# Accustomer/CUDA-AKAZE

Hardware: AMD Instinct MI355X
Metric: pairs_per_sec_detect_describe_match_1080p (higher is better)
Workload: dtype f32; 1 GPU; configs[1]: 1920x1080 grayscale pairs, 4 octaves x 4 sublevels, PM_G2, MLDB-486, max_pts 10000, float path; detect+describe both images + match, D2H included; pairs_per_launch_sequence=256, distinct_pairs_per_gpu=16, float_sequences_enqueued=77, octave_streams=one stream per context, step_pipeline=2, rank0_gpu_numa_node=1

## Files before the change

cuda-akaze_amd/akaze_hip/__init__.py:

```python
import ctypes as C
import os

import numpy as np

try:
    import torch as _torch
except ImportError:
    _torch = None

_HERE = os.path.dirname(os.path.abspath(__file__))
LIB_PATH = os.environ.get("HAK_LIB") or os.path.join(os.path.dirname(_HERE), "libhipakaze.so")

FLEN = 61
MAX_DIST = 96
PM_G1, PM_G2, WEICKERT, CHARBONNIER = 0, 1, 2, 3

POINT_DTYPE = np.dtype([
    ("x", "<f4"), ("y", "<f4"), ("octave", "<i4"), ("response", "<f4"), ("size", "<f4"), ("angle", "<f4"),
    ("features", "u1", (FLEN,)), ("_pad", "u1", (3,)),
    ("match", "<i4"), ("distance", "<i4"), ("match_x", "<f4"), ("match_y", "<f4"),
])
assert POINT_DTYPE.itemsize == 104
MATCH_PAIR_DTYPE = np.dtype([("query", "<i4"), ("train", "<i4"), ("distance", "<i4"), ("second", "<i4"),
                             ("x1", "<f4"), ("y1", "<f4"), ("x2", "<f4"), ("y2", "<f4")])
# ... 99 lines not shown
    "hak_memcpy_h2d": (C.c_int, [_vp, _vp, C.c_long]),
    "hak_fed_tau": (C.c_int, [C.c_float, C.c_int, C.c_float, C.c_int, _fp, C.c_int]),
    "hak_gauss_taps": (None, [C.c_float, C.c_int, _fp]),
    "hak_compare_indices": (None, [_ip, _ip]),
    "hak_describe_plan_query": (C.c_int, [C.c_int, C.POINTER(C.c_uint), C.POINTER(C.c_uint)]),
    "hak_query_schedule": (C.c_int, [_vp, _ip, _ip, _fp, _fp]),
    "hak_query_geometry": (C.c_int, [_vp, _ip]),
    "hak_query_traffic": (C.c_int, [_vp, C.c_int, C.POINTER(hak_traffic)]),
    "hak_prof_enable": (C.c_int, [_vp, C.c_int]),
    "hak_prof_read": (C.c_int, [_vp, C.c_int, C.POINTER(C.c_double), _ip]),
    "hak_prof_reset": (C.c_int, [_vp]),
}
TEST_SYMBOLS = {
    "hak_debug_plane": (C.c_int, [_vp, C.c_int, C.c_int, C.c_int, C.c_int, _vp]),
    "hak_debug_kcontrast": (C.c_int, [_vp, C.c_int, _fp]),
    "hak_op_lowpass": (C.c_int, [_vp, _vp, C.c_int, C.c_int, C.c_int, C.c_float, C.c_int]),
    "hak_op_down_smooth": (C.c_int, [_vp, _vp, _vp, C.c_int, C.c_int, C.c_int, C.c_int, C.c_int, C.c_int]),
    "hak_op_kcontrast": (C.c_int, [_vp, C.c_int, C.c_int, C.c_int, C.c_float, _fp, _fp, _ip]),
    "hak_op_flow": (C.c_int, [_vp, _vp, C.c_int, C.c_int, C.c_int, C.c_int, C.c_float]),
    "hak_op_nld_steps": (C.c_int, [_vp, _vp, _vp, _vp, C.c_int, C.c_int, C.c_int, _fp, C.c_int]),
    "hak_op_nld_steps_batch": (C.c_int, [_vp, _vp, _vp, _vp, C.c_long, C.c_int, C.c_int, C.c_int, C.c_int, _fp, C.c_int]),
    "hak_op_fed_cycle": (C.c_int, [_vp, C.c_int, C.c_int, C.c_int, C.c_int, _vp, _vp, _vp, _vp, C.c_long, C.c_int, C.c_int, C.c_int, C.c_int,
                                   _fp, _fp, C.c_int]),
    "hak_op_rcp_check": (C.c_int, [C.c_uint, C.c_uint, C.POINTER(C.c_ulonglong)]),
    "hak_op_smooth_flow": (C.c_int, [_vp, _vp, _vp, C.c_int, C.c_int, C.c_int, C.c_int, C.c_float]),
    "hak_op_hessian": (C.c_int, [_vp, _vp, _vp, _vp, C.c_int, C.c_int, C.c_int, C.c_int]),
    "hak_op_fast_conv_u8": (C.c_int, [_vp, C.c_int, _vp, C.c_int, C.c_int, C.c_int, C.c_float, C.c_int]),
    "hak_op_fast_lowpass": (C.c_int, [_vp, _vp, C.c_int, C.c_int, C.c_int, C.c_float, C.c_int]),
    "hak_op_fast_base": (C.c_int, [_vp, C.c_int, _vp, C.c_int, C.c_int, C.c_int, C.c_float, C.c_int, C.c_float, _ip, _ip, _ip, _ip]),
    "hak_op_fast_down_smooth": (C.c_int, [_vp, _vp, _vp, C.c_int, C.c_int, C.c_int, C.c_int, C.c_int, C.c_int]),
    "hak_op_fast_kcontrast": (C.c_int, [_vp, C.c_int, C.c_int, C.c_int, C.c_float, _ip, _ip, _ip]),
    "hak_op_fast_flow": (C.c_int, [_vp, _vp, C.c_int, C.c_int, C.c_int, C.c_int, C.c_int]),
    "hak_op_fast_smooth_flow": (C.c_int, [_vp, _vp, _vp, C.c_int, C.c_int, C.c_int, C.c_int, C.c_int]),
    "hak_op_fast_nld_steps": (C.c_int, [_vp, _vp, _vp, _vp, C.c_int, C.c_int, C.c_int, _fp, C.c_int]),
    "hak_op_fast_nld_steps_batch": (C.c_int, [_vp, _vp, _vp, _vp, C.c_long, C.c_int, C.c_int, C.c_int, C.c_int, _fp, C.c_int]),
    "hak_op_fast_fed_cycle": (C.c_int, [_vp, C.c_int, C.c_int, C.c_int, C.c_int, _vp, _vp, _vp, _vp, C.c_long, C.c_int, C.c_int, C.c_int,
                                        C.c_int, _ip, _fp, C.c_int]),
    "hak_op_fast_level_tile": (C.c_int, [_vp, C.c_int, C.c_int, C.c_int, C.c_int, _vp, _vp, _vp, C.c_long, C.c_int, C.c_int, C.c_int,
                                         C.c_int, C.c_int, _ip, _fp, C.c_int, _ip]),
    "hak_op_fast_hessian": (C.c_int, [_vp, _vp, _vp, _vp, C.c_int, C.c_int, C.c_int, C.c_int, _ip]),
    "hak_op_hessian_batch": (C.c_int, [_vp, _vp, _vp, _vp, C.c_int, C.c_int, C.c_int, C.c_int, C.c_int, _ip]),
    "hak_op_fast_hessian_batch": (C.c_int, [_vp, _vp, _vp, _vp, C.c_int, C.c_int, C.c_int, C.c_int, C.c_int, _ip]),
    "hak_debug_set_plane": (C.c_int, [_vp, C.c_int, C.c_int, C.c_int, C.c_int, _vp]),
    "hak_op_tail_begin": (C.c_int, [_vp]),
    "hak_op_tail_level": (C.c_int, [_vp, C.c_int, C.c_int, _vp]),
    "hak_op_tail_det_level": (C.c_int, [_vp, C.c_int, C.c_int, _vp]),
# ... 24 lines not shown


class _Libs:

    def __init__(self):
        self.product = C.CDLL(LIB_PATH, mode=C.RTLD_GLOBAL)
        self.test = None
        for name, (res, args) in SYMBOLS.items():
            try:
                f = getattr(self.product, name)
            except AttributeError:
                if os.environ.get("HAK_LIB"):
                    continue
                raise
            f.restype, f.argtypes = res, args
            setattr(self, name, f)

    def load_test(self):
        if self.test is None:
            if not os.path.exists(TEST_LIB_PATH):
                raise ImportError(f"{TEST_LIB_PATH} is missing: build it with `make -C cuda-akaze_amd/csrc`")
            self.test = C.CDLL(TEST_LIB_PATH)
            for name, (res, args) in TEST_SYMBOLS.items():
                f = getattr(self.test, name)
                f.restype, f.argtypes = res, args
                setattr(self, name, f)
        return self.test

    def __getattr__(self, name):
        if name in TEST_SYMBOLS:
            self.load_test()
            return self.__dict__[name]
        raise AttributeError(name)


lib = _Libs()


def check(status):
    if status != 0:
        raise HakError(lib.hak_last_error().decode() or f"libhipakaze status {status}")


def iAlignUp(a, b):
    return a - a % b + b if a % b else a


# ... 484 lines not shown
```

cuda-akaze_amd/csrc/hak_internal.h:

```cpp
#pragma once
#include <cstdlib>
#include <hip/hip_runtime.h>
#include <stdint.h>
#include "../../include/hipakaze.h"
#include "hak_knobs.h"

#define HAK_NBINS 300
#define HAK_WAVE 64

struct HakOct {
    int w, h, p;
    long plane;
};

struct HakLayout {
    int noct, ms;
    HakOct oct[HAK_MAX_OCTAVES];
    long lvl_off[HAK_MAX_OCTAVES];
    long smooth_off[HAK_MAX_OCTAVES], flow_off[HAK_MAX_OCTAVES], tmp_off[HAK_MAX_OCTAVES];
    long arena;

    __host__ __device__ long lt(int o, int s) const { return lvl_off[o] + (long)s * oct[o].plane; }
    __host__ __device__ long dxy(int o, int s) const { return lvl_off[o] + (long)(ms + 2 * s) * oct[o].plane; }
};
// ... 342 lines not shown
                          bool* hess_done = nullptr, float fixed_ikc = 0.f);
int hak_launch_level_tile(hipStream_t st, const int* src, HakOct so, bool head, int* smooth, int* dst, int* tmp, long stride,
                          HakOct dd, int nimg, const int* taps, int diffusivity, const float* tau, int n,
                          const HakImgState* state, int octave, int* dxy = nullptr, int step = 0, const HakBatch* b = nullptr,
                          const HakLayout* L = nullptr, const HakTables* htab = nullptr, int sub = 0, int idthreshold = 0, bool* hess_done = nullptr);
int hak_launch_rcp_check(unsigned lo, unsigned hi, unsigned long long* d_bad);
static inline bool hak_fed_sf_covers(const HakKnobs& kn, int diffusivity, const HakOct& dd, int nimg, const HakOct* so = nullptr)
{
    if (!hak_stream_pays(kn.fuse_sf, dd.w, dd.h, nimg) || diffusivity != HAK_PM_G2 || (dd.w & 3) != 0 || dd.w < 16 || dd.h < 8) return false;
    return !so || (kn.fuse_head && !(so->w & 1) && !(so->h & 1));
}
bool hak_launch_fed_sf_head(hipStream_t st, const float* src, HakOct so, float* smooth, float* flow, float* dst, long stride,
                            HakOct dd, int nimg, const float* taps, int diffusivity, const float* tau, int ns,
                            const HakImgState* state, int octave, bool write_g);
bool hak_launch_fed_sf_head(hipStream_t st, const int* src, HakOct so, int* smooth, int* flow, int* dst, long stride,
                            HakOct dd, int nimg, const int* taps, int diffusivity, const float* tau, int ns,
                            const HakImgState* state, int octave, bool write_g);
bool hak_launch_fed_sf(hipStream_t st, const float* src, float* smooth, float* flow, float* dst, long stride,
                       int w, int h, int p, int nimg, const float* taps, int diffusivity, const float* tau, int ns,
                       const HakImgState* state, int octave, bool write_g, bool store_smooth = true, float fixed_ikc = 0.f);
bool hak_launch_fed_sf(hipStream_t st, const int* src, int* smooth, int* flow, int* dst, long stride,
                       int w, int h, int p, int nimg, const int* taps, int diffusivity, const float* tau, int ns,
                       const HakImgState* state, int octave, bool write_g);
int hak_fed_groups(int n, int max_fuse, int w, bool wide_only);
bool hak_fed_wide_only(int octave, int w);
int hak_fed_group_size(int n, int G, int g);
void hak_launch_fed_group(hipStream_t st, const float* src, const float* flow, float* dst, long stride,
                          int w, int h, int p, int nimg, const float* tau, int ns);
void hak_launch_fed_group(hipStream_t st, const int* src, const int* flow, int* dst, long stride,
                          int w, int h, int p, int nimg, const float* tau, int ns);
void hak_launch_derivate(hipStream_t st, const float* src, float* dxy, long stride, int w, int h, int p, int nimg, int step);
void hak_launch_derivate(hipStream_t st, const int* src, int* dxy, long stride, int w, int h, int p, int nimg, int step);
void hak_launch_hessian(hipStream_t st, const float* dxy, float* det, long stride, int w, int h, int p, int nimg, int step);
void hak_launch_hessian(hipStream_t st, const int* dxy, int* det, long stride, int w, int h, int p, int nimg, int step);
void hak_deriv_factors(float* fac1, float* fac2);
template <typename V> static inline void hak_deriv_factors_as(V& f1, V& f2)
{
    float a, b;
    hak_deriv_factors(&a, &b);
    f1 = hak_fac_as(a, V());
    f2 = hak_fac_as(b, V());
}
void hak_launch_deinterleave(hipStream_t st, const float* ab, float* a, float* b, int w, int h, int p);

void hak_launch_ingest_u8(hipStream_t st, const unsigned char* src, long src_stride, int sp, float* dst, long dst_stride,
                          int dp, int w, int h, int nimg);
// ... 214 lines not shown
```

cuda-akaze_amd/csrc/hak_knobs.h:

```cpp
#pragma once
#include "../../include/hipakaze.h"

#define HAK_FED_MAX_FUSE 8

struct HakKnobs {
    int hess_stream = 1;
    int base_stream = 1;
    int base_hist = 0;
    int hess_cbuf = 256;
    int desc_order = 4;
    int desc_plan = 1;
    int desc_sort = 1;
    int hess_lp = 0;
    int level_tile = 1;
    int level_hess = 1;
    int level_min_steps = 8;
    int level_min_blocks = 96;
    int fuse_sf = 1;
    int fuse_head = 1;
    int max_fuse = 8;
    int hist_min_blocks = 256;
    int hist_rpb_max = 8;
    int hess_side = 0;
    int spine_max_px = 0;
    int side_streams = HAK_MAX_OCTAVES;
    int graph_pads = 1;
    int tail_fork = 1;
    int graph = 1;
    int serial = 0;
    int null_order = 1;
    int timing = 0;
    int prof_fence = 0;
    int stream_min_waves = 2048;
    int download_blocks = 128;
};
HakKnobs hak_knobs_from_env();
const HakKnobs& hak_process_knobs();

struct HakMatchKnobs {
    int valu = 0;
    int qt = 1;
    int slices = 0;
};
// ... 2 lines not shown
```

cuda-akaze_amd/csrc/hak_knobs.hip:

```cpp
#include "hak_knobs.h"
#include <climits>
#include <cstdlib>

static int env_int(const char* name, int dflt, int lo = INT_MIN, int hi = INT_MAX)
{
    const char* e = getenv(name);
    if (!e) return dflt;
    const long v = strtol(e, nullptr, 10);
    return v < lo ? lo : (v > hi ? hi : (int)v);
}

HakKnobs hak_knobs_from_env()
{
    static const struct { const char* name; int HakKnobs::*field; int lo, hi; } rows[] = {
        {"HAK_HESS_STREAM", &HakKnobs::hess_stream, INT_MIN, INT_MAX},
        {"HAK_BASE_STREAM", &HakKnobs::base_stream, INT_MIN, INT_MAX},
        {"HAK_BASE_HIST", &HakKnobs::base_hist, INT_MIN, INT_MAX},
        {"HAK_HESS_CBUF", &HakKnobs::hess_cbuf, 1, 256},
        {"HAK_DESC_ORDER", &HakKnobs::desc_order, 0, 255},
        {"HAK_DESC_PLAN", &HakKnobs::desc_plan, INT_MIN, INT_MAX},
        {"HAK_DESC_SORT", &HakKnobs::desc_sort, INT_MIN, INT_MAX},
        {"HAK_HESS_LP", &HakKnobs::hess_lp, INT_MIN, INT_MAX},
        {"HAK_LEVEL_TILE", &HakKnobs::level_tile, INT_MIN, INT_MAX},
        {"HAK_LEVEL_HESS", &HakKnobs::level_hess, INT_MIN, INT_MAX},
        {"HAK_LEVEL_MIN_STEPS", &HakKnobs::level_min_steps, INT_MIN, INT_MAX},
        {"HAK_LEVEL_MIN_BLOCKS", &HakKnobs::level_min_blocks, 1, INT_MAX},
        {"HAK_FUSE_SF", &HakKnobs::fuse_sf, INT_MIN, INT_MAX},
        {"HAK_FUSE_HEAD", &HakKnobs::fuse_head, INT_MIN, INT_MAX},
        {"HAK_FED_MAX_FUSE", &HakKnobs::max_fuse, 1, HAK_FED_MAX_FUSE},
        {"HAK_HIST_MIN_BLOCKS", &HakKnobs::hist_min_blocks, 1, INT_MAX},
        {"HAK_HIST_RPB_MAX", &HakKnobs::hist_rpb_max, 1, INT_MAX},
        {"HAK_HESS_SIDE", &HakKnobs::hess_side, INT_MIN, INT_MAX},
        {"HAK_SPINE_MAX_PX", &HakKnobs::spine_max_px, INT_MIN, INT_MAX},
        {"HAK_SIDE_STREAMS", &HakKnobs::side_streams, 1, INT_MAX},
        {"HAK_GRAPH_PADS", &HakKnobs::graph_pads, INT_MIN, INT_MAX},
        {"HAK_TAIL_FORK", &HakKnobs::tail_fork, INT_MIN, INT_MAX},
        {"HAK_GRAPH", &HakKnobs::graph, INT_MIN, INT_MAX},
        {"HAK_SERIAL", &HakKnobs::serial, INT_MIN, INT_MAX},
        {"HAK_NULL_ORDER", &HakKnobs::null_order, INT_MIN, INT_MAX},
        {"HAK_TIMING", &HakKnobs::timing, INT_MIN, INT_MAX},
        {"HAK_PROF_FENCE", &HakKnobs::prof_fence, INT_MIN, INT_MAX},
        {"HAK_STREAM_MIN_WAVES", &HakKnobs::stream_min_waves, 1, INT_MAX},
        {"HAK_DOWNLOAD_BLOCKS", &HakKnobs::download_blocks, 1, INT_MAX},
    };
    HakKnobs k;
    for (const auto& r : rows) k.*r.field = env_int(r.name, k.*r.field, r.lo, r.hi);
    return k;
}

const HakKnobs& hak_process_knobs()
{
    static const HakKnobs k = hak_knobs_from_env();
// ... 12 lines not shown
```

cuda-akaze_amd/csrc/hak_sequence.hip:

```cpp
#include "hak_internal.h"
#include <cstdio>
#include <cstring>
#include <string>
#include <type_traits>

#include "hak_ctx.h"

static thread_local const char* g_launch_err = nullptr;
void hak_note_launch_error(const char* msg) { if (!g_launch_err) g_launch_err = msg; }

void order_after_null_stream(hak_ctx* c, hipStream_t st)
{
    if (!c || !c->null_order || !c->ev_null || st == nullptr) return;
    const hipError_t q = hipStreamQuery(nullptr);
    if (q == hipSuccess) return;
    (void)hipGetLastError();
    if (hipEventRecord(c->ev_null, nullptr) != hipSuccess || hipStreamWaitEvent(st, c->ev_null, 0) != hipSuccess) (void)hipGetLastError();
}

void maps_guard_begin(hak_ctx* c)
{
    if (c->maps_dirty) {
        const size_t h = c->L.oct[0].h, words = (c->L.oct[0].w + 63) / 64, B = c->cfg.batch;
        (void)hipMemsetAsync(c->maps, 0, sizeof(unsigned long long) * (size_t)c->L.oct[0].plane * B, c->stream);
// ... 71 lines not shown
        const auto* img = static_cast<const std::conditional_t<is_fast<V>, unsigned char, float>*>(a.images);
        const V* taps_base = taps_of<V>(c->taps_base, c->itaps_base);
        const bool based = hak_launch_base_level(st, img, a.image_stride, a.pitch, Lt, tmp, S, oc.w, oc.h, oc.p, nimg, taps1, taps_base, c->base_R,
                                                 c->state, cfg.per, L.noct, kn);
        if constexpr (is_fast<V>) {
            if (!based) {
                hak_launch_lowpass(st, img, a.image_stride, a.pitch, smooth, S, oc.w, oc.h, oc.p, nimg, taps1, 2);
                hak_launch_contrast(st, smooth, S, oc.w, oc.h, oc.p, nimg, c->state, cfg.per, L.noct);
                hak_launch_lowpass(st, img, a.image_stride, a.pitch, Lt, S, oc.w, oc.h, oc.p, nimg, taps_base, c->base_R);
            }
        } else (void)based;
        return;
    }
    const int n = lp.nsteps;
    if (level_tile_pays(c, oc, nimg) && (is_fast<V> || s == 0 || n >= kn.level_min_steps || kn.level_tile == 2)) {
        ProfScope ps(pc, HAK_PROF_FED, st);
        const int nl = hak_launch_level_tile(st, s == 0 ? A + L.lt(o - 1, 0) : A + L.lt(o, s - 1), s == 0 ? L.oct[o - 1] : oc, s == 0, smooth, Lt, tmp, S,
                                             oc, nimg, taps1, cfg.diffusivity, lp.tau.data(), n, c->state, o,
                                             kn.level_hess ? A + L.dxy(o, s) : nullptr, lp.sigma_size, &a.b, &L, &c->htab, s, dthreshold_of<V>(c),
                                             &a.hess_fused[o * HAK_MAX_SCALES + s]);
        count_fed(nl, (s == 0 ? 1.0 * L.oct[o - 1].w * L.oct[o - 1].h : 4.0 * oc.w * oc.h) + 8.0 * oc.w * oc.h + (nl - 1) * 12.0 * oc.w * oc.h);
        return;
    }
    const int G = hak_fed_groups(n, is_fast<V> && kn.max_fuse > 4 ? 4 : kn.max_fuse, oc.w, hak_fed_wide_only(o, oc.w));
    const int ns0 = hak_fed_group_size(n, G, 0);
    V* dst0 = (G % 2 == 1) ? Lt : tmp;
    const V* fsrc;
    bool fused_first = false;
    if (s == 0) {
        if (hak_fed_sf_covers(kn, cfg.diffusivity, oc, nimg, &L.oct[o - 1])) {
            ProfScope ps(pc, HAK_PROF_FED, st);
            fused_first = hak_launch_fed_sf_head(st, A + L.lt(o - 1, 0), L.oct[o - 1], smooth, flow, dst0, S, oc, nimg, taps1, cfg.diffusivity,
                                                 lp.tau.data(), ns0, c->state, o, G > 1);
            if (fused_first) count_fed(1, 2.0 * L.oct[o - 1].w * L.oct[o - 1].h + (G > 1 ? 12.0 : 8.0) * oc.w * oc.h);
        }
        V* first = (G % 2 == 0) ? Lt : tmp;
        if (!fused_first) {
            { ProfScope ps(pc, HAK_PROF_DOWN, st);
              hak_launch_down_smooth(st, A + L.lt(o - 1, 0), first, smooth, S, L.oct[o - 1], oc, nimg, taps1); }
            ProfScope ps(pc, HAK_PROF_FLOW, st);
            hak_launch_flow(st, smooth, flow, S, oc.w, oc.h, oc.p, nimg, cfg.diffusivity, c->state, o);
        }
        fsrc = first;
    } else {
        fsrc = A + L.lt(o, s - 1);
        if (hak_fed_sf_covers(kn, cfg.diffusivity, oc, nimg)) {
// ... 253 lines not shown
```

cuda-akaze_amd/csrc/hak_test_api.hip:

```cpp
#include "hak_ctx.h"
#include "../../include/hipakaze_test.h"
#include <cmath>
#include <cstdio>
#include <cstring>
#include <type_traits>

extern "C" int hak_debug_plane(hak_ctx* c, int img, int kind, int o, int s, float* h_dst)
{
    if (!c || img < 0 || img >= c->cfg.batch || o < 0 || o >= c->L.noct || s < 0 || s >= c->L.ms) return fail("bad plane");
    const HakLayout& L = c->L;
    const HakOct oc = L.oct[o];
    HIP_TRY(hipStreamSynchronize(c->stream));
    const float* arena = c->arena + (long)img * L.arena;
    if (kind == HAK_PLANE_LT) {
        HIP_TRY(hipMemcpy2D(h_dst, sizeof(float) * oc.w, arena + L.lt(o, s), sizeof(float) * oc.p, sizeof(float) * oc.w, oc.h, hipMemcpyDeviceToHost));
        return 0;
    }
    float* tmp = nullptr;
    HIP_TRY(hipMalloc((void**)&tmp, sizeof(float) * 2 * (size_t)oc.plane));
    int rc = 0;
    const float* src = tmp;
    if (kind == HAK_PLANE_DET) {
        const int step = c->plan[(size_t)o * L.ms + s].sigma_size;
        if (c->last_fast) hak_launch_hessian(nullptr, reinterpret_cast<const int*>(arena + L.dxy(o, s)), reinterpret_cast<int*>(tmp), 0, oc.w, oc.h, oc.p, 1, step);
// ... 221 lines not shown
    if (nsteps < 1 || nimg < 1 || !kcontrast) return fail("nsteps < 1, nimg < 1 or no contrast factors");
    if (p % 4 || stride % 4 || (op_fast<V> && head && sp % 4)) return fail("pitch and stride must be multiples of 4");
    HakImgState* state = nullptr;
    if (op_state<V>(&state, kcontrast, nimg)) return 1;
    V taps[8];
    op_taps<V>(1.f, 2, taps);
    const int G = hak_fed_groups(nsteps, op_max_fuse<V>(), w, false);
    const int ns0 = hak_fed_group_size(nsteps, G, 0);
    V* dst0 = (G % 2 == 1) ? dst : tmp;
    int rc = 0;
    const bool ok = head ? hak_launch_fed_sf_head(nullptr, src, HakOct{sw, sh, sp, (long)sh * sp}, smooth, flow, dst0, stride,
                                                  HakOct{w, h, p, (long)h * p}, nimg, taps, HAK_PM_G2, tau, ns0, state, 0, G > 1)
                         : hak_launch_fed_sf(nullptr, src, smooth, flow, dst0, stride, w, h, p, nimg, taps, HAK_PM_G2, tau, ns0, state, 0, G > 1);
    if (!ok) rc = fail(std::string(who) + ": k_fed_sf does not cover this case");
    else op_fed_groups<V>(dst0, flow, dst, tmp, stride, w, h, p, nimg, tau, nsteps, G, 1, ns0);
    const hipError_t e = hipDeviceSynchronize();
    if (e != hipSuccess && !rc) rc = fail(std::string(who) + ": " + (op_fast<V> ? hipGetErrorString(e) : "kernel"));
    (void)hipFree(state);
    return rc;
}
extern "C" int hak_op_fed_cycle(const float* src, int head, int sw, int sh, int sp, float* smooth, float* flow, float* dst, float* tmp,
                                long stride, int w, int h, int p, int nimg, const float* kcontrast, const float* tau, int nsteps)
{ return fed_cycle_t("hak_op_fed_cycle", src, head, sw, sh, sp, smooth, flow, dst, tmp, stride, w, h, p, nimg, kcontrast, tau, nsteps); }
extern "C" int hak_op_fast_fed_cycle(const int* src, int head, int sw, int sh, int sp, int* smooth, int* flow, int* dst, int* tmp,
                                     long stride, int w, int h, int p, int nimg, const int* kcontrast, const float* tau, int nsteps)
{ return fed_cycle_t("hak_op_fast_fed_cycle", src, head, sw, sh, sp, smooth, flow, dst, tmp, stride, w, h, p, nimg, kcontrast, tau, nsteps); }

extern "C" int hak_op_fast_base(const unsigned char* img, int sp, int* lt, int w, int h, int p, float var_base, int radius, float per,
                                int* kc, int* hmax, int* hist, int* route)
{
    if (radius < 1 || radius > 5) return fail("radius must be 1..5");
    if (p % 4) return fail("pitch must be a multiple of 4");
    int taps1[8], tapsb[8];
    op_taps<int>(1.f, 2, taps1);
    op_taps<int>(var_base, radius, tapsb);
    const HakKnobs kn = hak_knobs_from_env();
    const size_t plane = (size_t)h * p;
    int* buf = nullptr;
    HIP_TRY(hipMalloc((void**)&buf, sizeof(int) * 3 * plane));
    HakImgState* st = nullptr;
    if (hipMalloc((void**)&st, sizeof(HakImgState)) != hipSuccess) { (void)hipFree(buf); return fail("state alloc"); }
    (void)hipMemset(st, 0, sizeof(HakImgState));
    hak_launch_reset_state(nullptr, st, 1);
    int *Lt = buf, *grad = buf + plane, *smooth = buf + 2 * plane;
    const bool based = hak_launch_base_level(nullptr, img, 0, sp, Lt, grad, 0, w, h, p, 1, taps1, tapsb, radius, st, per, 1, kn);
    if (!based) {
// ... 393 lines not shown
```

cuda-akaze_amd/csrc/kernels_fedsf.hip:

```cpp
#include "fed_common.h"

#ifndef HAK_FS_PD
#define HAK_FS_PD 3
#endif
#ifndef HAK_FS_PD_MAXNS
#define HAK_FS_PD_MAXNS 4
#endif

namespace {

template <typename V, int NS>
struct FsState {
    static constexpr int W = fed_lane_px(NS);
    using Px = FedPx<V, W>;
    static constexpr int GS = fed_gsum_slots(NS);
    static constexpr int UF = fed_unroll(NS);
    static constexpr int PD = NS <= HAK_FS_PD_MAXNS ? HAK_FS_PD : 3;
    Px Lr[6];
    Px Rp[6];
    Px Sm[3];
    V SmL[3], SmR[3];
    Px Lw[NS][2];
    Px Qw[NS][2];
    GHrow<V, W> GH[GS];
    Px GV[GS];
    Px gprev;
    Px Lq[PD];
};

template <bool DEC, typename V, int W>
__device__ __forceinline__ FedPx<V, W> fs_fetch(const V* __restrict__ L, const int row, const int lp, const int xl, const int sh)
{
    if constexpr (!DEC) return px_load<V, W>(L + (long)row * lp + xl);
    else {
        const V* r = L + (long)min(2 * row, sh - 1) * lp + min(2 * xl, lp - 2 * W);
        FedPx<V, W> o;
#pragma unroll
        for (int i = 0; i < W / 2; i++) {
            const FedPx<V, 4> a = px_load<V, 4>(r + 4 * i);
            o.e[2 * i] = a.e[0];
            o.e[2 * i + 1] = a.e[2];
        }
        return o;
    }
}

struct FsOut { __amdgpu_buffer_rsrc_t r; unsigned smo, go; };

template <typename V, int NS, int U, bool YEDGE, bool XE, bool WRITE_G, bool DEC, bool WRITE_SM>
__device__ __forceinline__ void fs_iter(FsState<V, NS>& S, const int t, const V* __restrict__ L, V* __restrict__ D, const int p,
                                        const int xl, const int x0, const int w, const int h, const int ybeg, const int yend,
                                        const bool owns, const FedFacs<V, NS>& fac, const SfTaps<V> kk, const float ikc,
                                        const int lp, const int sh, const FsOut& O)
{
    constexpr int W = FsState<V, NS>::W, GS = FsState<V, NS>::GS, PD = FsState<V, NS>::PD;
    using Px = FedPx<V, W>;
    const bool le = x0 == 0, re = x0 + W - 1 == w - 1;
    {
        const Px Lc = S.Lq[pmod(U, PD)];
        S.Lr[pmod(U, 6)] = Lc;
        S.Lq[pmod(U, PD)] = fs_fetch<DEC, V, W>(L, min(t + PD, h - 1), lp, xl, sh);
    }
    {
        const Px c = S.Lr[pmod(U, 6)];
        V a[W + 4];
        a[0] = wave_shr1(c.e[W - 2]); a[1] = wave_shr1(c.e[W - 1]);
#pragma unroll
        for (int j = 0; j < W; j++) a[2 + j] = c.e[j];
        a[W + 2] = wave_shl1(c.e[0]); a[W + 3] = wave_shl1(c.e[1]);
        if (XE) {
            a[1] = le ? a[3] : a[1];
            a[0] = le ? a[4] : a[0];
            if constexpr (!DEC) {
                a[W + 2] = re ? a[W] : a[W + 2];
                a[W + 3] = re ? a[W - 1] : a[W + 3];
            } else {
                a[W + 2] = re ? a[W + 1] : a[W + 2];
                a[W + 3] = re ? a[W] : a[W + 3];
            }
        }
        Px rp;
#pragma unroll
        for (int j = 0; j < W; j++) rp.e[j] = hak_conv5(a[j + 2], a[j + 1], a[j + 3], a[j], a[j + 4], kk);
        S.Rp[pmod(U, 6)] = rp;
        if (YEDGE) {
            S.Rp[pmod(U - 2, 6)] = px_sel(t == 1, rp, S.Rp[pmod(U - 2, 6)]);
            S.Rp[pmod(U - 4, 6)] = px_sel(t == 2, rp, S.Rp[pmod(U - 4, 6)]);
            if constexpr (!DEC) {
                S.Rp[pmod(U, 6)] = px_sel(t == h, S.Rp[pmod(U - 2, 6)], S.Rp[pmod(U, 6)]);
                S.Rp[pmod(U, 6)] = px_sel(t == h + 1, S.Rp[pmod(U - 4, 6)], S.Rp[pmod(U, 6)]);
            } else {
                S.Rp[pmod(U, 6)] = px_sel(t == h, S.Rp[pmod(U - 1, 6)], S.Rp[pmod(U, 6)]);
                S.Rp[pmod(U, 6)] = px_sel(t == h + 1, S.Rp[pmod(U - 3, 6)], S.Rp[pmod(U, 6)]);
            }
        }
    }
    {
        const int a = t - 2;
        const Px c = S.Rp[pmod(U - 2, 6)], u1 = S.Rp[pmod(U - 3, 6)], d1 = S.Rp[pmod(U - 1, 6)];
        const Px u2 = S.Rp[pmod(U - 4, 6)], d2 = S.Rp[pmod(U, 6)];
        Px sm;
#pragma unroll
        for (int j = 0; j < W; j++) sm.e[j] = hak_conv5(c.e[j], u1.e[j], d1.e[j], u2.e[j], d2.e[j], kk);
        if constexpr (WRITE_SM)
            px_buf_store_nt(O.r, O.smo + (a >= ybeg && a < yend ? (unsigned)(a * p) * (unsigned)sizeof(V) : HAK_BUF_OOB), sm);
        V sl = wave_shr1(sm.e[W - 1]), sr = wave_shl1(sm.e[0]);
        if (XE) {
            sl = le ? sm.e[1] : sl;
            sr = re ? sm.e[W - 2] : sr;
        }
        S.Sm[pmod(U, 3)] = sm; S.SmL[pmod(U, 3)] = sl; S.SmR[pmod(U, 3)] = sr;
        if (YEDGE && a == 1) { S.Sm[pmod(U - 2, 3)] = sm; S.SmL[pmod(U - 2, 3)] = sl; S.SmR[pmod(U - 2, 3)] = sr; }
        if (YEDGE && a == h) {
            S.Sm[pmod(U, 3)] = S.Sm[pmod(U - 2, 3)]; S.SmL[pmod(U, 3)] = S.SmL[pmod(U - 2, 3)]; S.SmR[pmod(U, 3)] = S.SmR[pmod(U - 2, 3)];
        }
    }
    const int tf = t - 3;
    {
        V su[W + 2], sc[W + 2], sd[W + 2];
        su[0] = S.SmL[pmod(U - 2, 3)]; su[W + 1] = S.SmR[pmod(U - 2, 3)];
        sc[0] = S.SmL[pmod(U - 1, 3)]; sc[W + 1] = S.SmR[pmod(U - 1, 3)];
        sd[0] = S.SmL[pmod(U, 3)]; sd[W + 1] = S.SmR[pmod(U, 3)];
#pragma unroll
        for (int j = 0; j < W; j++) {
            su[j + 1] = S.Sm[pmod(U - 2, 3)].e[j];
            sc[j + 1] = S.Sm[pmod(U - 1, 3)].e[j];
            sd[j + 1] = S.Sm[pmod(U, 3)].e[j];
        }
        float den[W];
        bool fast = true;
#pragma unroll
        for (int j = 0; j < W; j++) {
            V dx, dy;
            hak_scharr(su[j], su[j + 1], su[j + 2], sc[j], sc[j + 2], sd[j], sd[j + 1], sd[j + 2], dx, dy);
            den[j] = 1.f + hak_dif2(dx, dy, ikc);
            fast = fast && den[j] < 0x1p64f;
        }
        Px g;
        if (__ballot(!fast) == 0ull) {
#pragma unroll
            for (int j = 0; j < W; j++) g.e[j] = hak_g_as<V>(hak_rcp_newton(den[j]));
        } else {
#pragma unroll
            for (int j = 0; j < W; j++) g.e[j] = hak_g_as<V>(1.f / den[j]);
        }
        if (WRITE_G) px_buf_store_nt(O.r, O.go + (tf >= ybeg && tf < yend ? (unsigned)(tf * p) * (unsigned)sizeof(V) : HAK_BUF_OOB), g);
        S.GH[pmod(U, GS)] = fed_gh(g);
        S.GV[pmod(U - 1, GS)] = px_add(S.gprev, g);
        S.gprev = g;
    }
#pragma unroll
    for (int k = 1; k <= NS; k++) {
        const int rho = tf - k;
        const Px Lc = k == 1 ? S.Lr[pmod(U - 3 - 1, 6)] : S.Lw[k - 1][pmod(U - k, 2)];
        const Px Ls = k == 1 ? S.Lr[pmod(U - 3, 6)] : S.Lw[k - 1][pmod(U - k + 1, 2)];
        Px Qn = fed_q(S.GV[pmod(U - k, GS)], Ls, Lc);
        Px Qp = S.Qw[k - 1][pmod(U - k - 1, 2)];
        if (YEDGE) {
            Qp = px_sel(rho == 0, px_neg(Qn), Qp);
            Qn = px_sel(rho == h - 1, px_neg(Qp), Qn);
        }
        S.Qw[k - 1][pmod(U - k, 2)] = Qn;
        const Px out = fed_row<XE>(Lc, S.GH[pmod(U - k, GS)], Qn, Qp, x0, w, fac.f[k - 1]);
        if (k < NS) {
            S.Lw[k < NS ? k : 0][pmod(U - k, 2)] = out;
        } else if (rho >= ybeg && rho < yend && owns) {
            px_store_nt(D + (long)rho * p + x0, out);
        }
// ... 143 lines not shown
    return true;
}

__global__ __launch_bounds__(256) void k_rcp_check(unsigned lo, unsigned hi, unsigned long long* bad)
{
    unsigned long long n = 0;
    for (unsigned long long b = lo + blockIdx.x * (unsigned long long)blockDim.x + threadIdx.x; b < hi;
         b += (unsigned long long)gridDim.x * blockDim.x) {
        const float d = __uint_as_float((unsigned)b);
        n += __float_as_uint(hak_rcp_newton(d)) != __float_as_uint(1.0f / d);
    }
    if (n) atomicAdd(bad, n);
}

template <typename V>
bool launch_fed_sf_head_t(hipStream_t st, const V* src, HakOct so, V* smooth, V* flow, V* dst, long stride, HakOct dd, int nimg,
                          const V* taps, int diffusivity, const float* tau, int ns, const HakImgState* state, int octave, bool write_g)
{
    if ((so.w & 1) || (so.h & 1) || so.p < 2 * 8 || dd.w != so.w / 2 || dd.h != so.h / 2) return false;
    return launch_fs_any<V>(st, src, smooth, flow, dst, stride, dd.w, dd.h, dd.p, nimg, SfTaps<V>{taps[0], taps[1], taps[2]},
                            diffusivity, tau, ns, state, octave, 0.f, write_g, so.p, so.h);
}

}

int hak_launch_rcp_check(unsigned lo, unsigned hi, unsigned long long* d_bad)
{
    k_rcp_check<<<4096, 256>>>(lo, hi, d_bad);
    return hipGetLastError() == hipSuccess ? 0 : 1;
}

bool hak_launch_fed_sf(hipStream_t st, const float* src, float* smooth, float* flow, float* dst, long stride,
                       int w, int h, int p, int nimg, const float* taps, int diffusivity, const float* tau, int ns,
                       const HakImgState* state, int octave, bool write_g, bool store_smooth, float fixed_ikc)
{ return launch_fs_any<float>(st, src, store_smooth ? smooth : nullptr, flow, dst, stride, w, h, p, nimg, SfTaps<float>{taps[0], taps[1], taps[2]},
                                diffusivity, tau, ns, state, octave, fixed_ikc, write_g); }
bool hak_launch_fed_sf(hipStream_t st, const int* src, int* smooth, int* flow, int* dst, long stride,
                       int w, int h, int p, int nimg, const int* taps, int diffusivity, const float* tau, int ns,
                       const HakImgState* state, int octave, bool write_g)
{ return launch_fs_any<int>(st, src, smooth, flow, dst, stride, w, h, p, nimg, SfTaps<int>{taps[0], taps[1], taps[2]},
                              diffusivity, tau, ns, state, octave, 0.f, write_g); }

bool hak_launch_fed_sf_head(hipStream_t st, const float* src, HakOct so, float* smooth, float* flow, float* dst, long stride,
                            HakOct dd, int nimg, const float* taps, int diffusivity, const float* tau, int ns,
                            const HakImgState* state, int octave, bool write_g)
{ return launch_fed_sf_head_t<float>(st, src, so, smooth, flow, dst, stride, dd, nimg, taps, diffusivity, tau, ns, state, octave, write_g); }
bool hak_launch_fed_sf_head(hipStream_t st, const int* src, HakOct so, int* smooth, int* flow, int* dst, long stride,
                            HakOct dd, int nimg, const int* taps, int diffusivity, const float* tau, int ns,
                            const HakImgState* state, int octave, bool write_g)
{ return launch_fed_sf_head_t<int>(st, src, so, smooth, flow, dst, stride, dd, nimg, taps, diffusivity, tau, ns, state, octave, write_g); }
```

Measured before the change: 6484 pairs/s.

## Add whole-plane LDS-resident FED kernel for small octaves

Adds a kernel that runs an entire FED cycle (smoothing, conductivity, and all explicit diffusion steps) for one small image plane per workgroup. The plane stays in registers and LDS, and bands exchange halo rows through LDS instead of going through global memory across grouped launches. It is enabled by default for float path octaves up to 256 wide and 32K pixels when the batch has at least 128 images. This removes multiple launches and global round trips at coarse octaves, at the cost of one block per image, high register pressure, and large LDS use.

```diff
diff --git a/cuda-akaze_amd/akaze_hip/__init__.py b/cuda-akaze_amd/akaze_hip/__init__.py
--- a/cuda-akaze_amd/akaze_hip/__init__.py
+++ b/cuda-akaze_amd/akaze_hip/__init__.py
@@ -145,6 +145,9 @@
     "hak_op_nld_steps_batch": (C.c_int, [_vp, _vp, _vp, _vp, C.c_long, C.c_int, C.c_int, C.c_int, C.c_int, _fp, C.c_int]),
     "hak_op_fed_cycle": (C.c_int, [_vp, C.c_int, C.c_int, C.c_int, C.c_int, _vp, _vp, _vp, _vp, C.c_long, C.c_int, C.c_int, C.c_int, C.c_int,
                                    _fp, _fp, C.c_int]),
+    "hak_op_fed_cycle_plane": (C.c_int, [_vp, C.c_int, C.c_int, C.c_int, C.c_int, _vp, _vp, _vp, _vp, C.c_long, C.c_int, C.c_int, C.c_int,
+                                         C.c_int, _fp, _fp, C.c_int]),
+    "hak_op_fed_plane_pays": (C.c_int, [C.c_int, C.c_int, C.c_int]),
     "hak_op_rcp_check": (C.c_int, [C.c_uint, C.c_uint, C.POINTER(C.c_ulonglong)]),
     "hak_op_smooth_flow": (C.c_int, [_vp, _vp, _vp, C.c_int, C.c_int, C.c_int, C.c_int, C.c_float]),
     "hak_op_hessian": (C.c_int, [_vp, _vp, _vp, _vp, C.c_int, C.c_int, C.c_int, C.c_int]),
@@ -215,7 +218,12 @@
                 raise ImportError(f"{TEST_LIB_PATH} is missing: build it with `make -C cuda-akaze_amd/csrc`")
             self.test = C.CDLL(TEST_LIB_PATH)
             for name, (res, args) in TEST_SYMBOLS.items():
-                f = getattr(self.test, name)
+                try:
+                    f = getattr(self.test, name)
+                except AttributeError:
+                    if os.environ.get("HAK_LIB"):
+                        continue
+                    raise
                 f.restype, f.argtypes = res, args
                 setattr(self, name, f)
         return self.test
diff --git a/cuda-akaze_amd/csrc/hak_internal.h b/cuda-akaze_amd/csrc/hak_internal.h
--- a/cuda-akaze_amd/csrc/hak_internal.h
+++ b/cuda-akaze_amd/csrc/hak_internal.h
@@ -388,6 +388,17 @@
 bool hak_launch_fed_sf(hipStream_t st, const int* src, int* smooth, int* flow, int* dst, long stride,
                        int w, int h, int p, int nimg, const int* taps, int diffusivity, const float* tau, int ns,
                        const HakImgState* state, int octave, bool write_g);
+#define HAK_FED_PLANE_ROWS 9
+#define HAK_FED_PLANE_MAX_PX 32768
+#define HAK_FED_PLANE_MIN_IMAGES 128
+static inline bool hak_fed_plane_covers(int w, int h)
+{
+    return (w & 3) == 0 && w >= 8 && w <= 256 && h >= 8 && h <= 16 * HAK_FED_PLANE_ROWS && (long)w * h <= HAK_FED_PLANE_MAX_PX;
+}
+static inline bool hak_fed_plane_pays(int w, int h, int nimg) { return hak_fed_plane_covers(w, h) && nimg >= HAK_FED_PLANE_MIN_IMAGES; }
+bool hak_launch_fed_plane(hipStream_t st, const float* src, HakOct so, bool head, float* smooth, float* dst, long stride, HakOct dd,
+                          int nimg, const float* taps, int diffusivity, const float* tau, int n, const HakImgState* state, int octave,
+                          float fixed_ikc = 0.f);
 int hak_fed_groups(int n, int max_fuse, int w, bool wide_only);
 bool hak_fed_wide_only(int octave, int w);
 int hak_fed_group_size(int n, int G, int g);
diff --git a/cuda-akaze_amd/csrc/hak_knobs.h b/cuda-akaze_amd/csrc/hak_knobs.h
--- a/cuda-akaze_amd/csrc/hak_knobs.h
+++ b/cuda-akaze_amd/csrc/hak_knobs.h
@@ -19,6 +19,7 @@
     int fuse_sf = 1;
     int fuse_head = 1;
     int max_fuse = 8;
+    int fed_plane = 1;
     int hist_min_blocks = 256;
     int hist_rpb_max = 8;
     int hess_side = 0;
diff --git a/cuda-akaze_amd/csrc/hak_knobs.hip b/cuda-akaze_amd/csrc/hak_knobs.hip
--- a/cuda-akaze_amd/csrc/hak_knobs.hip
+++ b/cuda-akaze_amd/csrc/hak_knobs.hip
@@ -28,6 +28,7 @@
         {"HAK_FUSE_SF", &HakKnobs::fuse_sf, INT_MIN, INT_MAX},
         {"HAK_FUSE_HEAD", &HakKnobs::fuse_head, INT_MIN, INT_MAX},
         {"HAK_FED_MAX_FUSE", &HakKnobs::max_fuse, 1, HAK_FED_MAX_FUSE},
+        {"HAK_FED_PLANE", &HakKnobs::fed_plane, 0, 2},
         {"HAK_HIST_MIN_BLOCKS", &HakKnobs::hist_min_blocks, 1, INT_MAX},
         {"HAK_HIST_RPB_MAX", &HakKnobs::hist_rpb_max, 1, INT_MAX},
         {"HAK_HESS_SIDE", &HakKnobs::hess_side, INT_MIN, INT_MAX},
diff --git a/cuda-akaze_amd/csrc/hak_sequence.hip b/cuda-akaze_amd/csrc/hak_sequence.hip
--- a/cuda-akaze_amd/csrc/hak_sequence.hip
+++ b/cuda-akaze_amd/csrc/hak_sequence.hip
@@ -117,6 +117,16 @@
         count_fed(nl, (s == 0 ? 1.0 * L.oct[o - 1].w * L.oct[o - 1].h : 4.0 * oc.w * oc.h) + 8.0 * oc.w * oc.h + (nl - 1) * 12.0 * oc.w * oc.h);
         return;
     }
+    if constexpr (!is_fast<V>) {
+        if (kn.fed_plane == 2 ? hak_fed_plane_covers(oc.w, oc.h) : (kn.fed_plane == 1 && hak_fed_plane_pays(oc.w, oc.h, nimg))) {
+            ProfScope ps(pc, HAK_PROF_FED, st);
+            if (hak_launch_fed_plane(st, s == 0 ? A + L.lt(o - 1, 0) : A + L.lt(o, s - 1), s == 0 ? L.oct[o - 1] : oc, s == 0, smooth, Lt, S, oc,
+                                     nimg, taps1, cfg.diffusivity, lp.tau.data(), n, c->state, o)) {
+                count_fed(1, (s == 0 ? 2.0 * L.oct[o - 1].w * L.oct[o - 1].h : 4.0 * oc.w * oc.h) + 8.0 * oc.w * oc.h);
+                return;
+            }
+        }
+    }
     const int G = hak_fed_groups(n, is_fast<V> && kn.max_fuse > 4 ? 4 : kn.max_fuse, oc.w, hak_fed_wide_only(o, oc.w));
     const int ns0 = hak_fed_group_size(n, G, 0);
     V* dst0 = (G % 2 == 1) ? Lt : tmp;
diff --git a/cuda-akaze_amd/csrc/hak_test_api.hip b/cuda-akaze_amd/csrc/hak_test_api.hip
--- a/cuda-akaze_amd/csrc/hak_test_api.hip
+++ b/cuda-akaze_amd/csrc/hak_test_api.hip
@@ -267,6 +267,23 @@
 extern "C" int hak_op_fed_cycle(const float* src, int head, int sw, int sh, int sp, float* smooth, float* flow, float* dst, float* tmp,
                                 long stride, int w, int h, int p, int nimg, const float* kcontrast, const float* tau, int nsteps)
 { return fed_cycle_t("hak_op_fed_cycle", src, head, sw, sh, sp, smooth, flow, dst, tmp, stride, w, h, p, nimg, kcontrast, tau, nsteps); }
+extern "C" int hak_op_fed_cycle_plane(const float* src, int head, int sw, int sh, int sp, float* smooth, float* flow, float* dst, float* tmp,
+                                      long stride, int w, int h, int p, int nimg, const float* kcontrast, const float* tau, int nsteps)
+{
+    (void)flow; (void)tmp;
+    if (nsteps < 1 || nimg < 1 || !kcontrast) return fail("nsteps < 1, nimg < 1 or no contrast factors");
+    HakImgState* state = nullptr;
+    if (op_state<float>(&state, kcontrast, nimg)) return 1;
+    float taps[8];
+    op_taps<float>(1.f, 2, taps);
+    if (!hak_launch_fed_plane(nullptr, src, head ? HakOct{sw, sh, sp, (long)sh * sp} : HakOct{w, h, p, (long)h * p}, head != 0, smooth, dst, stride,
+                              HakOct{w, h, p, (long)h * p}, nimg, taps, HAK_PM_G2, tau, nsteps, state, 0)) {
+        (void)hipFree(state);
+        return fail("hak_op_fed_cycle_plane: k_fed_sf_plane does not cover this case");
+    }
+    return op_sync_free("hak_op_fed_cycle_plane", state);
+}
+extern "C" int hak_op_fed_plane_pays(int w, int h, int nimg) { return hak_fed_plane_pays(w, h, nimg) ? 1 : 0; }
 extern "C" int hak_op_fast_fed_cycle(const int* src, int head, int sw, int sh, int sp, int* smooth, int* flow, int* dst, int* tmp,
                                      long stride, int w, int h, int p, int nimg, const int* kcontrast, const float* tau, int nsteps)
 { return fed_cycle_t("hak_op_fast_fed_cycle", src, head, sw, sh, sp, smooth, flow, dst, tmp, stride, w, h, p, nimg, kcontrast, tau, nsteps); }
diff --git a/cuda-akaze_amd/csrc/kernels_fedsf.hip b/cuda-akaze_amd/csrc/kernels_fedsf.hip
--- a/cuda-akaze_amd/csrc/kernels_fedsf.hip
+++ b/cuda-akaze_amd/csrc/kernels_fedsf.hip
@@ -1,3 +1,4 @@
+#include <atomic>
 #include "fed_common.h"
 
 #ifndef HAK_FS_PD
@@ -45,6 +46,62 @@
     }
 }
 
+template <bool DEC, bool XE, typename V, int W>
+__device__ __forceinline__ FedPx<V, W> fs_row_pass(const FedPx<V, W>& c, const bool le, const bool re, const SfTaps<V>& kk)
+{
+    V a[W + 4];
+    a[0] = wave_shr1(c.e[W - 2]); a[1] = wave_shr1(c.e[W - 1]);
+#pragma unroll
+    for (int j = 0; j < W; j++) a[2 + j] = c.e[j];
+    a[W + 2] = wave_shl1(c.e[0]); a[W + 3] = wave_shl1(c.e[1]);
+    if (XE) {
+        a[1] = le ? a[3] : a[1];
+        a[0] = le ? a[4] : a[0];
+        if constexpr (!DEC) {
+            a[W + 2] = re ? a[W] : a[W + 2];
+            a[W + 3] = re ? a[W - 1] : a[W + 3];
+        } else {
+            a[W + 2] = re ? a[W + 1] : a[W + 2];
+            a[W + 3] = re ? a[W] : a[W + 3];
+        }
+    }
+    FedPx<V, W> rp;
+#pragma unroll
+    for (int j = 0; j < W; j++) rp.e[j] = hak_conv5(a[j + 2], a[j + 1], a[j + 3], a[j], a[j + 4], kk);
+    return rp;
+}
+template <bool XE, typename V, int W>
+__device__ __forceinline__ void fs_sm_sides(const FedPx<V, W>& sm, const bool le, const bool re, V& sl, V& sr)
+{
+    sl = wave_shr1(sm.e[W - 1]); sr = wave_shl1(sm.e[0]);
+    if (XE) {
+        sl = le ? sm.e[1] : sl;
+        sr = re ? sm.e[W - 2] : sr;
+    }
+}
+template <typename V, int W>
+__device__ __forceinline__ FedPx<V, W> fs_conductivity(const V (&su)[W + 2], const V (&sc)[W + 2], const V (&sd)[W + 2], const float ikc)
+{
+    float den[W];
+    bool fast = true;
+#pragma unroll
+    for (int j = 0; j < W; j++) {
+        V dx, dy;
+        hak_scharr(su[j], su[j + 1], su[j + 2], sc[j], sc[j + 2], sd[j], sd[j + 1], sd[j + 2], dx, dy);
+        den[j] = 1.f + hak_dif2(dx, dy, ikc);
+        fast = fast && den[j] < 0x1p64f;
+    }
+    FedPx<V, W> g;
+    if (__ballot(!fast) == 0ull) {
+#pragma unroll
+        for (int j = 0; j < W; j++) g.e[j] = hak_g_as<V>(hak_rcp_newton(den[j]));
+    } else {
+#pragma unroll
+        for (int j = 0; j < W; j++) g.e[j] = hak_g_as<V>(1.f / den[j]);
+    }
+    return g;
+}
+
 struct FsOut { __amdgpu_buffer_rsrc_t r; unsigned smo, go; };
 
 template <typename V, int NS, int U, bool YEDGE, bool XE, bool WRITE_G, bool DEC, bool WRITE_SM>
@@ -62,26 +119,7 @@
         S.Lq[pmod(U, PD)] = fs_fetch<DEC, V, W>(L, min(t + PD, h - 1), lp, xl, sh);
     }
     {
-        const Px c = S.Lr[pmod(U, 6)];
-        V a[W + 4];
-        a[0] = wave_shr1(c.e[W - 2]); a[1] = wave_shr1(c.e[W - 1]);
-#pragma unroll
-        for (int j = 0; j < W; j++) a[2 + j] = c.e[j];
-        a[W + 2] = wave_shl1(c.e[0]); a[W + 3] = wave_shl1(c.e[1]);
-        if (XE) {
-            a[1] = le ? a[3] : a[1];
-            a[0] = le ? a[4] : a[0];
-            if constexpr (!DEC) {
-                a[W + 2] = re ? a[W] : a[W + 2];
-                a[W + 3] = re ? a[W - 1] : a[W + 3];
-            } else {
-                a[W + 2] = re ? a[W + 1] : a[W + 2];
-                a[W + 3] = re ? a[W] : a[W + 3];
-            }
-        }
-        Px rp;
-#pragma unroll
-        for (int j = 0; j < W; j++) rp.e[j] = hak_conv5(a[j + 2], a[j + 1], a[j + 3], a[j], a[j + 4], kk);
+        const Px rp = fs_row_pass<DEC, XE>(S.Lr[pmod(U, 6)], le, re, kk);
         S.Rp[pmod(U, 6)] = rp;
         if (YEDGE) {
             S.Rp[pmod(U - 2, 6)] = px_sel(t == 1, rp, S.Rp[pmod(U - 2, 6)]);
@@ -104,11 +142,8 @@
         for (int j = 0; j < W; j++) sm.e[j] = hak_conv5(c.e[j], u1.e[j], d1.e[j], u2.e[j], d2.e[j], kk);
         if constexpr (WRITE_SM)
             px_buf_store_nt(O.r, O.smo + (a >= ybeg && a < yend ? (unsigned)(a * p) * (unsigned)sizeof(V) : HAK_BUF_OOB), sm);
-        V sl = wave_shr1(sm.e[W - 1]), sr = wave_shl1(sm.e[0]);
-        if (XE) {
-            sl = le ? sm.e[1] : sl;
-            sr = re ? sm.e[W - 2] : sr;
-        }
+        V sl, sr;
+        fs_sm_sides<XE>(sm, le, re, sl, sr);
         S.Sm[pmod(U, 3)] = sm; S.SmL[pmod(U, 3)] = sl; S.SmR[pmod(U, 3)] = sr;
         if (YEDGE && a == 1) { S.Sm[pmod(U - 2, 3)] = sm; S.SmL[pmod(U - 2, 3)] = sl; S.SmR[pmod(U - 2, 3)] = sr; }
         if (YEDGE && a == h) {
@@ -127,23 +162,7 @@
             sc[j + 1] = S.Sm[pmod(U - 1, 3)].e[j];
             sd[j + 1] = S.Sm[pmod(U, 3)].e[j];
         }
-        float den[W];
-        bool fast = true;
-#pragma unroll
-        for (int j = 0; j < W; j++) {
-            V dx, dy;
-            hak_scharr(su[j], su[j + 1], su[j + 2], sc[j], sc[j + 2], sd[j], sd[j + 1], sd[j + 2], dx, dy);
-            den[j] = 1.f + hak_dif2(dx, dy, ikc);
-            fast = fast && den[j] < 0x1p64f;
-        }
-        Px g;
-        if (__ballot(!fast) == 0ull) {
-#pragma unroll
-            for (int j = 0; j < W; j++) g.e[j] = hak_g_as<V>(hak_rcp_newton(den[j]));
-        } else {
-#pragma unroll
-            for (int j = 0; j < W; j++) g.e[j] = hak_g_as<V>(1.f / den[j]);
-        }
+        const Px g = fs_conductivity<V, W>(su, sc, sd, ikc);
         if (WRITE_G) px_buf_store_nt(O.r, O.go + (tf >= ybeg && tf < yend ? (unsigned)(tf * p) * (unsigned)sizeof(V) : HAK_BUF_OOB), g);
         S.GH[pmod(U, GS)] = fed_gh(g);
         S.GV[pmod(U - 1, GS)] = px_add(S.gprev, g);
@@ -333,6 +352,154 @@
                             diffusivity, tau, ns, state, octave, 0.f, write_g, so.p, so.h);
 }
 
+constexpr int FP_R = HAK_FED_PLANE_ROWS;
+constexpr int FP_MAX_STEPS = 96;
+struct FpFacs { float f[FP_MAX_STEPS]; };
+constexpr int FP_LDS_MAX = HAK_FED_PLANE_MAX_PX * 4;
+
+template <bool DEC>
+__global__ __launch_bounds__(1024) void k_fed_sf_plane(const float* __restrict__ src, float* __restrict__ smooth, float* __restrict__ dst,
+                                                       long stride, int w, int h, int p, FpFacs fac, int ns, SfTaps<float> kk,
+                                                       const HakImgState* __restrict__ state, int octave, float fixed_ikc, int lp, int sh)
+{
+    using Px = FedPx<float, 4>;
+    extern __shared__ __align__(16) unsigned char fp_lds_raw[];
+    float* const P = reinterpret_cast<float*>(fp_lds_raw);
+    Px* const X = reinterpret_cast<Px*>(fp_lds_raw);
+    const int img = blockIdx.x;
+    const float* L0 = src + (long)img * stride;
+    float* SMO = smooth + (long)img * stride;
+    float* D = dst + (long)img * stride;
+    const float ikc = state ? state[img].ikc[octave] : fixed_ikc;
+    const int lane = threadIdx.x & 63;
+    const int band = __builtin_amdgcn_readfirstlane(threadIdx.x >> 6);
+    const int nb = blockDim.x >> 6;
+    const int x0 = 4 * lane, r0 = band * FP_R;
+    const int xl = min(x0, w - 4);
+    const bool col = x0 < w;
+    const bool le = x0 == 0, re = x0 + 3 == w - 1;
+    auto refl_lp = [&](int r) { return DEC ? hak_refl(2 * r, sh) >> 1 : hak_refl(r, h); };
+    auto lds_row = [&](int r) { return *reinterpret_cast<const Px*>(P + r * w + xl); };
+    auto lds_put = [&](int r, const Px& v) { if (col && r < h) *reinterpret_cast<Px*>(P + r * w + x0) = v; };
+
+    Px Lr[FP_R];
+#pragma unroll
+    for (int i = 0; i < FP_R; i++) Lr[i] = fs_fetch<DEC, float, 4>(L0, min(r0 + i, h - 1), lp, xl, sh);
+#pragma unroll
+    for (int i = 0; i < FP_R; i++) lds_put(r0 + i, fs_row_pass<DEC, true>(Lr[i], le, re, kk));
+    hak_lds_barrier();
+    Px Sm[FP_R + 2];
+    {
+        Px e[FP_R + 4];
+#pragma unroll
+        for (int k = 0; k < FP_R + 4; k++) e[k] = lds_row(refl_lp(r0 - 2 + k));
+#pragma unroll
+        for (int i = 0; i < FP_R; i++) {
+            Px sm;
+#pragma unroll
+            for (int j = 0; j < 4; j++) sm.e[j] = hak_conv5(e[i + 2].e[j], e[i + 1].e[j], e[i + 3].e[j], e[i].e[j], e[i + 4].e[j], kk);
+            Sm[i + 1] = sm;
+            if (col && r0 + i < h) px_store_nt(SMO + (long)(r0 + i) * p + x0, sm);
+        }
+    }
+    hak_lds_barrier();
+#pragma unroll
+    for (int i = 0; i < FP_R; i++) lds_put(r0 + i, Sm[i + 1]);
+    hak_lds_barrier();
+    Sm[0] = lds_row(hak_refl(r0 - 1, h));
+    Sm[FP_R + 1] = lds_row(hak_refl(r0 + FP_R, h));
+    if (r0 + FP_R > h) {
+#pragma unroll
+        for (int i = 1; i < FP_R; i++) Sm[i + 1] = px_sel(r0 + i >= h, lds_row(hak_refl(r0 + i, h)), Sm[i + 1]);
+    }
+    Px G[FP_R];
+    {
+        float su[6], sc[6], sd[6];
+        fs_sm_sides<true>(Sm[0], le, re, sc[0], sc[5]);
+        fs_sm_sides<true>(Sm[1], le, re, sd[0], sd[5]);
+#pragma unroll
+        for (int j = 0; j < 4; j++) { sc[j + 1] = Sm[0].e[j]; sd[j + 1] = Sm[1].e[j]; }
+#pragma unroll
+        for (int i = 0; i < FP_R; i++) {
+#pragma unroll
+            for (int j = 0; j < 6; j++) { su[j] = sc[j]; sc[j] = sd[j]; }
+            fs_sm_sides<true>(Sm[i + 2], le, re, sd[0], sd[5]);
+#pragma unroll
+            for (int j = 0; j < 4; j++) sd[j + 1] = Sm[i + 2].e[j];
+            G[i] = fs_conductivity<float, 4>(su, sc, sd, ikc);
+        }
+    }
+    hak_lds_barrier();
+    lds_put(r0, G[0]);
+    lds_put(r0 + FP_R - 1, G[FP_R - 1]);
+    hak_lds_barrier();
+    const Px gv_up = px_add(lds_row(max(r0 - 1, 0)), G[0]);
+    const Px g_dn = lds_row(min(r0 + FP_R, h - 1));
+    hak_lds_barrier();
+    Px* const GX = X + 2 * nb * 128 + band * 128 + lane;
+    GX[0] = gv_up;
+    GX[64] = g_dn;
+    const bool yedge = r0 == 0 || r0 + FP_R >= h;
+    const int up = max(band - 1, 0), dn = min(band + 1, nb - 1);
+    auto step_row = [&](const int i, const Px& Gn, const Px& Ln, Px& Qp, const bool ye, const float f) __attribute__((always_inline)) {
+        Px Qn = fed_q(px_add(G[i], Gn), Ln, Lr[i]);
+        if (ye) {
+            Qp = px_sel(r0 + i == 0, px_neg(Qn), Qp);
+            Qn = px_sel(r0 + i == h - 1, px_neg(Qp), Qn);
+        }
+        Lr[i] = fed_row<true>(Lr[i], fed_gh(G[i]), Qn, Qp, x0, w, f);
+        Qp = Qn;
+        __builtin_amdgcn_sched_barrier(0);
+    };
+    auto step = [&](const Px* buf, const bool ye, const float f) __attribute__((always_inline)) {
+        Px Qp = fed_q(GX[0], Lr[0], buf[up * 128 + 64 + lane]);
+#pragma unroll
+        for (int i = 0; i + 1 < FP_R; i++) step_row(i, G[i + 1], Lr[i + 1], Qp, ye, f);
+        step_row(FP_R - 1, GX[64], buf[dn * 128 + lane], Qp, ye, f);
+    };
+    for (int k = 0; k < ns; k++) {
+        Px* const buf = X + (k & 1) * nb * 128;
+        buf[band * 128 + lane] = Lr[0];
+        buf[band * 128 + 64 + lane] = Lr[FP_R - 1];
+        hak_lds_barrier();
+#pragma unroll
+        for (int i = 0; i < FP_R; i++)
+#pragma unroll
+            for (int j = 0; j < 4; j++) asm volatile("" : "+v"(G[i].e[j]));
+        if (yedge) step(buf, true, fac.f[k]);
+        else step(buf, false, fac.f[k]);
+    }
+#pragma unroll
+    for (int i = 0; i < FP_R; i++)
+        if (col && r0 + i < h) px_store_nt(D + (long)(r0 + i) * p + x0, Lr[i]);
+}
+
+bool launch_fed_plane(hipStream_t st, const float* src, HakOct so, bool head, float* smooth, float* dst, long stride, HakOct dd, int nimg,
+                      const float* taps, int diffusivity, const float* tau, int n, const HakImgState* state, int octave, float fixed_ikc)
+{
+    if (!hak_fed_plane_covers(dd.w, dd.h) || diffusivity != HAK_PM_G2 || n < 1 || n > FP_MAX_STEPS || nimg < 1) return false;
+    if (head && ((so.w & 1) || (so.h & 1) || so.p < 2 * 8 || (so.p & 3) || dd.w != so.w / 2 || dd.h != so.h / 2)) return false;
+    if ((dd.p & 3) || (stride & 3) || dd.p < dd.w) return false;
+    FpFacs fac;
+    for (int k = 0; k < FP_MAX_STEPS; k++) fac.f[k] = k < n ? 0.5f * tau[k] : 0.f;
+    const SfTaps<float> kk{taps[0], taps[1], taps[2]};
+    const int nb = (dd.h + FP_R - 1) / FP_R;
+    const size_t plane = sizeof(float) * (size_t)dd.w * dd.h, bufs = (size_t)nb * 6144;
+    const size_t lds = plane > bufs ? plane : bufs;
+    static std::atomic<unsigned long long> attr_done[2];
+    int dev = 0;
+    (void)hipGetDevice(&dev);
+    const unsigned long long bit = 1ull << (dev & 63);
+    if (!(attr_done[head].load(std::memory_order_acquire) & bit)) {
+        const void* fn = head ? reinterpret_cast<const void*>(&k_fed_sf_plane<true>) : reinterpret_cast<const void*>(&k_fed_sf_plane<false>);
+        (void)hipFuncSetAttribute(fn, hipFuncAttributeMaxDynamicSharedMemorySize, FP_LDS_MAX);
+        attr_done[head].fetch_or(bit, std::memory_order_release);
+    }
+    if (head) k_fed_sf_plane<true><<<nimg, 64 * nb, lds, st>>>(src, smooth, dst, stride, dd.w, dd.h, dd.p, fac, n, kk, state, octave, fixed_ikc, so.p, so.h);
+    else k_fed_sf_plane<false><<<nimg, 64 * nb, lds, st>>>(src, smooth, dst, stride, dd.w, dd.h, dd.p, fac, n, kk, state, octave, fixed_ikc, dd.p, dd.h);
+    return true;
+}
+
 }
 
 int hak_launch_rcp_check(unsigned lo, unsigned hi, unsigned long long* d_bad)
@@ -352,6 +519,11 @@
 { return launch_fs_any<int>(st, src, smooth, flow, dst, stride, w, h, p, nimg, SfTaps<int>{taps[0], taps[1], taps[2]},
                               diffusivity, tau, ns, state, octave, 0.f, write_g); }
 
+bool hak_launch_fed_plane(hipStream_t st, const float* src, HakOct so, bool head, float* smooth, float* dst, long stride, HakOct dd,
+                          int nimg, const float* taps, int diffusivity, const float* tau, int n, const HakImgState* state, int octave,
+                          float fixed_ikc)
+{ return launch_fed_plane(st, src, so, head, smooth, dst, stride, dd, nimg, taps, diffusivity, tau, n, state, octave, fixed_ikc); }
+
 bool hak_launch_fed_sf_head(hipStream_t st, const float* src, HakOct so, float* smooth, float* flow, float* dst, long stride,
                             HakOct dd, int nimg, const float* taps, int diffusivity, const float* tau, int ns,
                             const HakImgState* state, int octave, bool write_g)
```

New measurement: 6524 pairs/s, median of 6. Within noise of the previous version (+0.6%).
